# Tianion/topazdb

Hardware: AMD Instinct MI355X
Metric: GiB/s device-resident SSTable block decode+checksum, 4KiB blocks, 1 MI355X (higher is better)
Workload: dtype u8; 1 GPU; 4k: 1048576 blocks/GPU x 4155 B median, 34.0 entries/block, tag 1 (Uncompress); blocks_per_gpu=1048576, input_bytes_per_gpu=4356833280, parallelism=shard1

## Files before the change

### topazdb_amd/csrc/tpz_decode.hip

```cpp

#include <hip/hip_runtime.h>
#include <stdint.h>

#include "tpz_internal.h"
#include "tpz_spill.hip"

namespace tpz {

typedef uint32_t u32;
typedef uint64_t u64;

constexpr int kWave = 64;
#ifdef TPZ_ABL_W20
#ifdef TPZ_ABL_W8
constexpr int kWavesPerWG = 8;
#else
constexpr int kWavesPerWG = 10;
#endif
#else
constexpr int kWavesPerWG = 16;
#endif
constexpr int kWGThreads = kWave * kWavesPerWG;
constexpr u32 kRowShift = 4, kRowBlocks = 1u << kRowShift;
#ifndef TPZ_ROW_AHEAD
// ... 45 lines not shown

__device__ __forceinline__ u32 lane_id() {
  u32 l = __builtin_amdgcn_mbcnt_hi(~0u, __builtin_amdgcn_mbcnt_lo(~0u, 0u));
  asm volatile("" : "+v"(l));
  return l;
}
__device__ __forceinline__ u32 uni(u32 x) { return __builtin_amdgcn_readfirstlane(x); }
__device__ __forceinline__ u64 uni64(u64 x) {
  u32 lo = __builtin_amdgcn_readfirstlane((u32)x), hi = __builtin_amdgcn_readfirstlane((u32)(x >> 32));
  return ((u64)hi << 32) | lo;
}
__device__ __forceinline__ u32 readlane(u32 x, int l) { return __builtin_amdgcn_readlane(x, l); }
template <int CTRL>
__device__ __forceinline__ u32 dpp(u32 x) {
  return (u32)__builtin_amdgcn_update_dpp(0, (int)x, CTRL, 0xF, 0xF, true);
}
constexpr int kRowShr = 0x110;
constexpr int kRowShl = 0x100;

__device__ __forceinline__ u32 lds_u32(const uint8_t* base, u32 a) {
  const u32* p = reinterpret_cast<const u32*>(base + (a & ~3u));
  return __builtin_amdgcn_alignbyte(p[1], p[0], a & 3u);
}
__device__ __forceinline__ u32 lds_be16(const uint8_t* base, u32 a) {
  u32 w = lds_u32(base, a);
  return ((w & 0xFFu) << 8) | ((w >> 8) & 0xFFu);
}
__device__ __forceinline__ u32 bswap32(u32 w) { return __builtin_bswap32(w); }

__device__ __forceinline__ uint4 lds_window16(const uint8_t* base, int x) {
  typedef u32 u32x2 __attribute__((ext_vector_type(2)));
  const u32x2* p = reinterpret_cast<const u32x2*>(base + (x & ~7));
  u32x2 a = p[0], b = p[1], c = p[2];
  asm volatile("" : "+v"(a), "+v"(b), "+v"(c));
  const u32 s = (u32)x & 3u;
  const bool h = ((u32)x & 4u) != 0;
  const u32 s0 = h ? a.y : a.x, s1 = h ? b.x : a.y, s2 = h ? b.y : b.x, s3 = h ? c.x : b.y,
            s4 = h ? c.y : c.x;
  return make_uint4(__builtin_amdgcn_alignbyte(s1, s0, s), __builtin_amdgcn_alignbyte(s2, s1, s),
                    __builtin_amdgcn_alignbyte(s3, s2, s), __builtin_amdgcn_alignbyte(s4, s3, s));
}

#ifdef TPZ_ABL_NOCF
__device__ __forceinline__ u32 tlook(const u32* tab, int id, u32 byte) {
  u32 z = byte;
  asm volatile("" : "+v"(z));
  return tab[id * 256 + (((z & 0x10000u) + __builtin_amdgcn_mbcnt_lo(~0u, 0u)) & 31u)];
}
#elif defined(TPZ_ABL_W20)
__device__ __forceinline__ u32 tlook(const u32* tab, int id, u32 byte) { return tab[(id & 15) * 256 + byte]; }
#else
__device__ __forceinline__ u32 tlook(const u32* tab, int id, u32 byte) { return tab[id * 256 + byte]; }
#endif

__device__ __forceinline__ u32 xor3(u32 a, u32 b, u32 c) { return __builtin_amdgcn_bitop3_b32(a, b, c, 0x96); }

__device__ __forceinline__ u32 slice16(const u32* tab, u32 w0, u32 w1, u32 w2, u32 w3) {
  u32 c = xor3(tlook(tab, 15, w0 & 0xFF), tlook(tab, 14, (w0 >> 8) & 0xFF), tlook(tab, 13, (w0 >> 16) & 0xFF));
  c = xor3(c, tlook(tab, 12, w0 >> 24), tlook(tab, 11, w1 & 0xFF));
  c = xor3(c, tlook(tab, 10, (w1 >> 8) & 0xFF), tlook(tab, 9, (w1 >> 16) & 0xFF));
  c = xor3(c, tlook(tab, 8, w1 >> 24), tlook(tab, 7, w2 & 0xFF));
  c = xor3(c, tlook(tab, 6, (w2 >> 8) & 0xFF), tlook(tab, 5, (w2 >> 16) & 0xFF));
  c = xor3(c, tlook(tab, 4, w2 >> 24), tlook(tab, 3, w3 & 0xFF));
  c = xor3(c, tlook(tab, 2, (w3 >> 8) & 0xFF), tlook(tab, 1, (w3 >> 16) & 0xFF));
  return c ^ tlook(tab, 0, w3 >> 24);
}

__device__ __forceinline__ u32 crc_shift_small(const u32* tab, u32 a, u32 k) {
  u32 r = k >= 4 ? 0u : (a >> (8 * k));
  for (u32 i = 0; i < 4 && i < k; i++) r ^= tlook(tab, (int)(k - 1 - i), (a >> (8 * i)) & 0xFF);
  return r;
}

__device__ __forceinline__ u32 crc_unshift_small(const u32* tab, u32 r, u32 k) {
#ifdef TPZ_ABL_W20
  return r;
#endif
  for (u32 i = 0; i < k; i++) {
    const u32 b = tlook(tab, kCrcInvTable, r >> 24);
    r = ((r ^ tlook(tab, 0, b)) << 8) | b;
  }
  return r;
}

__device__ __forceinline__ u32 gf_mul(u32 a, u32 b) {
  u32 p = 0;
#pragma unroll
  for (int i = 0; i < 32; i++) {
    p ^= (a & (0x80000000u >> i)) ? b : 0u;
    b = (b >> 1) ^ ((b & 1u) ? 0xEDB88320u : 0u);
  }
  return p;
}

__device__ __forceinline__ u32 gf_mul_lane(u32 a, u32 b) {
  u32 p = 0;
#pragma unroll
  for (int i = 0; i < 32; i++) {
    const u32 m = (u32)((int)(a << i) >> 31);
    p ^= b & m;
    b = (b >> 1) ^ (0xEDB88320u & (u32)(-(int)(b & 1u)));
  }
  return p;
}

__device__ __forceinline__ u32 wave_xor(u32 x) {
  x ^= (u32)__builtin_amdgcn_update_dpp(0, (int)x, 0x100 + 1, 0xF, 0xF, true);
  x ^= (u32)__builtin_amdgcn_update_dpp(0, (int)x, 0x100 + 2, 0xF, 0xF, true);
  x ^= (u32)__builtin_amdgcn_update_dpp(0, (int)x, 0x100 + 4, 0xF, 0xF, true);
  x ^= (u32)__builtin_amdgcn_update_dpp(0, (int)x, 0x100 + 8, 0xF, 0xF, true);
  return __builtin_amdgcn_readlane(x, 0) ^ __builtin_amdgcn_readlane(x, 16) ^
         __builtin_amdgcn_readlane(x, 32) ^ __builtin_amdgcn_readlane(x, 48);
}

template <int J>
__device__ __forceinline__ u32 crc_shift(const u32* tab, u32 a) {
  constexpr int b0 = 16 + 4 * J;
  return xor3(tlook(tab, b0, a & 0xFF), tlook(tab, b0 + 1, (a >> 8) & 0xFF),
              tlook(tab, b0 + 2, (a >> 16) & 0xFF)) ^ tlook(tab, b0 + 3, a >> 24);
}

__device__ __forceinline__ uint4 keep_head(uint4 v, u32 k) {
  const u64 lo = (u64)v.y << 32 | v.x, hi = (u64)v.w << 32 | v.z;
  const u64 mlo = k >= 8 ? ~0ull : ((1ull << (8 * k)) - 1);
  const u64 mhi = k >= 16 ? ~0ull : (k <= 8 ? 0ull : ((1ull << (8 * (k - 8))) - 1));
  const u64 a = lo & mlo, b = hi & mhi;
  return make_uint4((u32)a, (u32)(a >> 32), (u32)b, (u32)(b >> 32));
}

__device__ __forceinline__ uint4 zero_head(uint4 v, u32 k) {
  const u64 lo = (u64)v.y << 32 | v.x, hi = (u64)v.w << 32 | v.z;
  const u64 mlo = k >= 8 ? 0ull : (~0ull << (8 * k));
  const u64 mhi = k <= 8 ? ~0ull : (~0ull << (8 * (k - 8)));
  const u64 a = lo & mlo, b = hi & mhi;
  return make_uint4((u32)a, (u32)(a >> 32), (u32)b, (u32)(b >> 32));
}

__device__ __forceinline__ u32 crc_combine(const u32* tab, u32 A) {
  u32 lane = lane_id();
  asm volatile("" : "+v"(lane));
  if ((lane & 1u) == 1u) A = crc_shift<0>(tab, A);
  A ^= dpp<kRowShl + 1>(A);
  if ((lane & 3u) == 2u) A = crc_shift<1>(tab, A);
  A ^= dpp<kRowShl + 2>(A);
  if ((lane & 7u) == 4u) A = crc_shift<2>(tab, A);
  A ^= dpp<kRowShl + 4>(A);
  if ((lane & 15u) == 8u) A = crc_shift<3>(tab, A);
  A ^= dpp<kRowShl + 8>(A);
  if ((lane & 31u) == 16u) A = crc_shift<4>(tab, A);
  if ((lane & 47u) == 32u) A = crc_shift<5>(tab, A);
  return readlane(A, 0) ^ readlane(A, 16) ^ readlane(A, 32) ^ readlane(A, 48);
}

__device__ __forceinline__ u32 wave_crc(const u32* tab, const uint8_t* win, int pb, u32 Pa) {
  typedef u32 u32x4 __attribute__((ext_vector_type(4)));
  const u32 lane = lane_id();
  const u32 S = (Pa + 5119) / 5120;
  u32 A = 0;
  for (u32 r = S; r-- > 0;) {
    const int seg = (int)Pa - 5120 * (int)r - kCrcLaneBytes * (int)(lane + 1);
    u32 c = 0;
    if (seg + kCrcLaneBytes > 0) {
#pragma unroll
      for (int t = 0; t < kCrcLaneBytes / 16; t++) {
        const u32x4 w = *reinterpret_cast<const u32x4*>(win + pb + seg + 16 * t);
        c = slice16(tab, w.x ^ c, w.y, w.z, w.w);
// ... 243 lines not shown
  const u32 vch = V ? (dv + V + 15) >> 4 : 0u;
  D.rk = __builtin_amdgcn_make_buffer_rsrc(o.keys + (kf & ~15ull), (short)0, (int)(16 * kch), 0x00020000);
  D.rv = __builtin_amdgcn_make_buffer_rsrc(o.vals + (vf & ~15ull), (short)0, (int)(16 * vch), 0x00020000);
  const u32 vs = 16 * kch + dv;
  D.rgk = dk | (dk + K) << 16;
  D.rgv = vs | (vs + V) << 16;
  return D;
}
template <bool FLAT>
__device__ __forceinline__ u32 stream_vstart(u32 K, u32 dk, u32 dv) {
  return FLAT ? (K ? (dk + K + 15) & ~15u : 0u) + dv : (K + 15) & ~15u;
}
struct FlatDst {
  static constexpr bool kFlat = true;
  const FlatOut* d;
  __device__ __forceinline__ void put(u32 c, uint4 acc, bool act) const { d->put(c, acc, !act); }
};

template <class Col, class MapT, class S, class D>
__device__ __forceinline__ u32 copy_window(const S& src, const Col& col, const MapT* map, u32 nk,
                                           u32 tot, const D& dst, u32 map_len, u32 w, u32 carry) {
  const u32 nch = (tot + 15) >> 4;
  const u32 lane = lane_id();
  const u32 last = nk ? nk - 1 : 0u;
  const u32 c = 64 * w + lane;
  const u32 x0 = 16 * c;
  const bool act = c < nch;
  u32 j = map[min(c, map_len - 1)];
  j = max(wave_scan_max(act ? j : 0u), carry);
  const u32 carry_out = readlane(j, 63);
  u32 e0, e1;
  int d0, d1;
  col.get2(min(j, last), e0, d0, e1, d1);
  uint4 acc = src(act ? (int)x0 + d0 : 0);
  bool cross = act && j + 1 < nk && e0 < x0 + 16;
  uint4 nx = make_uint4(0, 0, 0, 0);
  if (cross) nx = src((int)x0 + d1);
  if (__ballot(act && e0 <= x0)) {
    while (act && e0 <= x0 && (!D::kFlat || j < last)) {
      j++;
      col.get2(min(j, last), e0, d0, e1, d1);
    }
    acc = src(act ? (int)x0 + d0 : 0);
    cross = act && j + 1 < nk && e0 < x0 + 16;
    if (cross) nx = src((int)x0 + d1);
  }
  if (cross) acc = merge_at(acc, nx, (int)(e0 - x0));
  if (__ballot(cross && e1 < x0 + 16 && j + 2 < nk)) {
    u32 k = j + 1, end = e1;
    while (cross && end < x0 + 16 && k + 1 < nk) {
      const int lo = (int)(end - x0);
      k++;
      int delta;
      col.get(k, end, delta);
      const int hi = min((int)(end - x0), 16);
      const uint4 v = src((int)x0 + delta);
      acc.x = (acc.x & ~byte_mask(lo, hi, 0)) | (v.x & byte_mask(lo, hi, 0));
      acc.y = (acc.y & ~byte_mask(lo, hi, 1)) | (v.y & byte_mask(lo, hi, 1));
      acc.z = (acc.z & ~byte_mask(lo, hi, 2)) | (v.z & byte_mask(lo, hi, 2));
      acc.w = (acc.w & ~byte_mask(lo, hi, 3)) | (v.w & byte_mask(lo, hi, 3));
    }
  }
  dst.put(c, acc, act);
  return carry_out;
}

template <class Col, class MapT, class S, class D>
__device__ __forceinline__ void copy_stream(const S& src, const Col& col, const MapT* map, u32 nk,
                                            u32 tot, const D& dst, u32 map_len) {
  const u32 lane = lane_id();
  const u32 nch = (tot + 15) >> 4;
  const u32 npad = (nch + 7) & ~7u;
  const u32 nw = (npad + 63) >> 6;
#ifdef TPZ_ABL_MEMONLY
  for (u32 c = lane; c < npad; c += 64) dst.put(c, make_uint4(c, 0, 0, 0), c < nch);
  return;
#endif
  u32 carry = 0;
  for (u32 w = 0; w < nw; w++) carry = copy_window(src, col, map, nk, tot, dst, map_len, w, carry);
}

struct PendingCrc {
  u32 live;
  u32 b, st, cnt, stored, k;
  u32 lc;
  u32 early;
};

__device__ __forceinline__ void finish_pending(const u32* tab, const Out& o, PendingCrc& pd) {
  if (!pd.live) return;
  const u32 R = crc_combine(tab, pd.lc);
  const u32 crc = (R == crc_shift_small(tab, ~pd.stored, pd.k)) ? pd.stored
                                                                   : ~crc_unshift_small(tab, R, pd.k);
  const bool ok = crc == pd.stored;
  put_meta(o, pd.b, ok ? pd.st : TPZ_BLOCK_CHECKSUM_MISMATCH, ok ? pd.cnt : 0u, crc);
  pd.live = 0;
}

struct FinishAtExit {
  const u32* tab;
  const Out& o;
  PendingCrc& pd;
  bool on;
  __device__ __forceinline__ ~FinishAtExit() {
    if (on) finish_pending(tab, o, pd);
  }
};

template <int J>
__device__ __forceinline__ bool comb_lane(u32 lane) {
  return J == 0 ? (lane & 1u) == 1u : J == 1 ? (lane & 3u) == 2u : J == 2 ? (lane & 7u) == 4u
       : J == 3 ? (lane & 15u) == 8u : J == 4 ? (lane & 31u) == 16u : (lane & 47u) == 32u;
}
struct CombLv {
  u32 r0, r1, r2, r3;
};
template <int J>
__device__ __forceinline__ CombLv comb_issue(const u32* tab, u32 A) {
  CombLv c;
  if (comb_lane<J>(lane_id())) {
    constexpr int b0 = 16 + 4 * J;
    c.r0 = tlook(tab, b0, A & 0xFF);
    c.r1 = tlook(tab, b0 + 1, (A >> 8) & 0xFF);
    c.r2 = tlook(tab, b0 + 2, (A >> 16) & 0xFF);
    c.r3 = tlook(tab, b0 + 3, A >> 24);
  }
  return c;
}
template <int J>
__device__ __forceinline__ u32 comb_use(u32 A, const CombLv& c) {
  if (comb_lane<J>(lane_id())) A = xor3(c.r0, c.r1, c.r2) ^ c.r3;
  if (J < 4) A ^= dpp<kRowShl + (1 << (J < 4 ? J : 0))>(A);
  return A;
}

__device__ __forceinline__ void comb_finish(const u32* tab, const Out& o, PendingCrc& pd, u32 cA,
                                            u32 want) {
  if (!pd.live) return;
  const u32 R = readlane(cA, 0) ^ readlane(cA, 16) ^ readlane(cA, 32) ^ readlane(cA, 48);
  const u32 crc = R == want ? pd.stored : ~crc_unshift_small(tab, R, pd.k);
  const bool ok = crc == pd.stored;
  put_meta(o, pd.b, ok ? pd.st : TPZ_BLOCK_CHECKSUM_MISMATCH, ok ? pd.cnt : 0u, crc);
  pd.live = 0;
}

struct CrcLane {
  int seg;
  bool act;
  u32 c;
};

__device__ __forceinline__ void crc_step(const u32* tab, const uint8_t* win, int pb, CrcLane& L,
                                         int t) {
  typedef u32 u32x4 __attribute__((ext_vector_type(4)));
  const int a = L.act ? pb + L.seg + 16 * t : -kGuard;
  const u32x4 w = *reinterpret_cast<const u32x4*>(win + a);
  L.c = slice16(tab, w.x ^ L.c, w.y, w.z, w.w);
}
__device__ __forceinline__ u32 crc_lane_value(const u32* tab, const CrcLane& L) { return L.c; }

struct FastWin {
  u32 nk, tot, nch, npad, last;
  __amdgpu_buffer_rsrc_t out;
};

template <bool FLAT, class S>
__device__ __forceinline__ u32 copy_fast(const S& src, const ColSmall& col, const uint16_t* map,
                                         const FastWin& F, const FlatOut& D, u32 w, u32 carry,
                                         u32& rare) {
  const u32 lane = lane_id();
  const u32 c = 64 * w + lane;
  const u32 x0 = 16 * c;
  const bool act = c < F.nch;
  u32 j = map[min(c, (u32)kWaveMapLen - 1)];
  j = max(wave_scan_max(act ? j : 0u), carry);
  const u32 carry_out = readlane(j, 63);
  u32 e0, e1;
  int d0, d1;
  col.get2(min(j, F.last), e0, d0, e1, d1);
  const bool cross = act && j + 1 < F.nk && e0 < x0 + 16;
  uint4 acc = src(act ? (int)x0 + d0 : -kGuard);
  const uint4 nx = src(cross ? (int)x0 + d1 : -kGuard);
  const bool rw = __ballot(act && (e0 <= x0 || (cross && e1 < x0 + 16 && j + 2 < F.nk))) != 0;
  if (rw) rare |= 1u << w;
  if (cross) acc = merge_at(acc, nx, (int)(e0 - x0));
  if (FLAT) {
    D.put(c, acc, rw);
  } else {
    __builtin_amdgcn_raw_buffer_store_b128(__builtin_bit_cast(__attribute__((ext_vector_type(4))) u32, acc),
                                           F.out, rw ? kOob : x0, 0, 0);
  }
  return carry_out;
}

template <bool FLAT, class S>
__device__ __forceinline__ u32 copy_fast3(const S& src, const ColSmall& col, const uint16_t* map,
                                          const FastWin& F, const FlatOut& D, u32 w, u32 carry,
                                          u32& rare) {
  const u32 lane = lane_id();
  const u32 c = 64 * w + lane;
  const u32 x0 = 16 * c;
  const bool act = c < F.nch;
  u32 j = map[min(c, (u32)kWaveMapLen - 1)];
  j = max(wave_scan_max(act ? j : 0u), carry);
  const u32 carry_out = readlane(j, 63);
  u32 e0, e1, e2, e3;
  int d0, d1, d2, d3;
  col.get2(min(j, F.last), e0, d0, e1, d1);
  col.get2(min(j + 2, F.last), e2, d2, e3, d3);
  if (act && e0 <= x0) {
    j++;
    e0 = e1, d0 = d1, e1 = e2, d1 = d2, e2 = e3, d2 = d3;
  }
  const bool b1 = act && j + 1 < F.nk && e0 < x0 + 16;
  const bool b2 = b1 && j + 2 < F.nk && e1 < x0 + 16;
  uint4 acc = src(act ? (int)x0 + d0 : -kGuard);
  const uint4 n1 = src(b1 ? (int)x0 + d1 : -kGuard);
  const uint4 n2 = src(b2 ? (int)x0 + d2 : -kGuard);
  const bool rw = __ballot(act && (e0 <= x0 || (b2 && e2 < x0 + 16 && j + 3 < F.nk))) != 0;
  if (rw) rare |= 1u << w;
  if (b1) acc = merge_at(acc, n1, (int)(e0 - x0));
  if (b2) acc = merge_at(acc, n2, (int)(e1 - x0));
  if (FLAT)
    D.put(c, acc, rw);
  else
    __builtin_amdgcn_raw_buffer_store_b128(__builtin_bit_cast(__attribute__((ext_vector_type(4))) u32, acc),
                                           F.out, rw ? kOob : x0, 0, 0);
  return carry_out;
}

template <bool SHORT, bool FLAT, class S>
__device__ __forceinline__ u32 copy_crc_fused(const u32* tab, const S& src, const ColSmall& col,
                                              const uint16_t* map, u32 nk, u32 tot, uint8_t* dst,
                                              const FlatOut& D, const uint8_t* win, int pb, u32 Pa,
                                              u32 kshift, Stamps& St, u32 w3, const Out& o,
                                              PendingCrc& pd) {
  const u32 lane = lane_id();
  FastWin F;
  F.nk = nk;
  F.tot = tot;
  F.nch = (tot + 15) >> 4;
  F.npad = FLAT ? F.nch : (F.nch + 7) & ~7u;
  F.last = nk ? nk - 1 : 0u;
  F.out = __builtin_amdgcn_make_buffer_rsrc(dst, (short)0, FLAT ? 0 : (int)(F.npad * 16), 0x00020000);
  const u32 nw = (F.npad + 63) >> 6;
  CrcLane L;
  L.seg = (int)Pa - kCrcLaneBytes * (int)(lane + 1);
  L.act = L.seg + kCrcLaneBytes > 0;
  L.c = 0;
  u32 carry = 0, rare = 0, cw[5];
  const bool pl = pd.live != 0;
  u32 cA = pd.lc, want = 0;
  CombLv cl{0u, 0u, 0u, 0u};
  if (pl) {
    cl = comb_issue<0>(tab, cA);
    want = crc_shift_small(tab, ~pd.stored, pd.k);
  }
#pragma unroll
  for (int t = 0; t < 4; t++) {
    cw[t] = carry;
    crc_step(tab, win, pb, L, t);
    carry = (SHORT && (u32)t < w3) ? copy_fast3<FLAT>(src, col, map, F, D, (u32)t, carry, rare)
                                   : copy_fast<FLAT>(src, col, map, F, D, (u32)t, carry, rare);
    if (pl) {
      if (t == 0) { cA = comb_use<0>(cA, cl); cl = comb_issue<1>(tab, cA); }
      if (t == 1) { cA = comb_use<1>(cA, cl); cl = comb_issue<2>(tab, cA); }
      if (t == 2) { cA = comb_use<2>(cA, cl); cl = comb_issue<3>(tab, cA); }
      if (t == 3) { cA = comb_use<3>(cA, cl); cl = comb_issue<4>(tab, cA); }
    }
  }
  cw[4] = carry;
  crc_step(tab, win, pb, L, 4);
  if (pl) {
    cA = comb_use<4>(cA, cl);
    cl = comb_issue<5>(tab, cA);
  }
  if (nw > 4)
    carry = (SHORT && 4u < w3) ? copy_fast3<FLAT>(src, col, map, F, D, 4u, carry, rare)
                               : copy_fast<FLAT>(src, col, map, F, D, 4u, carry, rare);
  if (pl) comb_finish(tab, o, pd, comb_use<5>(cA, cl), want);
  TPZ_STAMP(St, 4);
#ifdef TPZ_ABL_STAMPS
  St.rare += __builtin_popcount(rare);
#endif
  if (rare) {
    for (u32 w = 0; w < nw; w++)
      if (rare & (1u << w)) {
        if (FLAT)
          copy_window(src, col, map, nk, F.tot, FlatDst{&D}, (u32)kWaveMapLen, w, cw[w]);
        else
          copy_window(src, col, map, nk, F.tot, SlotDst{dst, F.npad, F.tot}, (u32)kWaveMapLen, w, cw[w]);
      }
  }
  return crc_lane_value(tab, L);
}

typedef u32 u32x2v __attribute__((ext_vector_type(2)));
typedef u32 u32x4v __attribute__((ext_vector_type(4)));
struct Gath {
  u32 d0, d1, d2, d3, d4;
};
__device__ __forceinline__ Gath gath_issue(const uint8_t* base, int x) {
  const u32* p = reinterpret_cast<const u32*>(base + (x & ~3));
  Gath g;
  g.d0 = p[0];
  g.d1 = p[1];
  g.d2 = p[2];
  g.d3 = p[3];
  g.d4 = p[4];
  return g;
}
__device__ __forceinline__ uint4 gath_finish(Gath g, int x) {
  asm volatile("" : "+v"(g.d0), "+v"(g.d1), "+v"(g.d2), "+v"(g.d3), "+v"(g.d4));
  const u32 s = (u32)x & 3u;
  return make_uint4(__builtin_amdgcn_alignbyte(g.d1, g.d0, s), __builtin_amdgcn_alignbyte(g.d2, g.d1, s),
                    __builtin_amdgcn_alignbyte(g.d3, g.d2, s), __builtin_amdgcn_alignbyte(g.d4, g.d3, s));
}
struct Look16 {
  u32 r[16];
};
__device__ __forceinline__ Look16 look_issue(const u32* tab, u32x4v w, u32 c) {
  Look16 L;
  const u32 w0 = w.x ^ c;
#pragma unroll
  for (int i = 0; i < 4; i++) {
    L.r[i] = tlook(tab, 15 - i, (w0 >> (8 * i)) & 0xFF);
    L.r[4 + i] = tlook(tab, 11 - i, (w.y >> (8 * i)) & 0xFF);
    L.r[8 + i] = tlook(tab, 7 - i, (w.z >> (8 * i)) & 0xFF);
    L.r[12 + i] = tlook(tab, 3 - i, (w.w >> (8 * i)) & 0xFF);
  }
  return L;
}
__device__ __forceinline__ u32 look_xor(const Look16& L) {
  u32 c = xor3(L.r[0], L.r[1], L.r[2]);
  c = xor3(c, L.r[3], L.r[4]);
  c = xor3(c, L.r[5], L.r[6]);
  c = xor3(c, L.r[7], L.r[8]);
  c = xor3(c, L.r[9], L.r[10]);
  c = xor3(c, L.r[11], L.r[12]);
  c = xor3(c, L.r[13], L.r[14]);
  return c ^ L.r[15];
}
#define TPZ_SB() __builtin_amdgcn_sched_barrier(0)

struct PWin {
  u32 m, j;
  u32 e0, e1;
  int d0, d1;
  bool act, cross;
  Gath ga, gn;
};
struct PWin3 {
  u32 e2, e3;
  int d2, d3;
  bool b2;
  Gath g2;
};

struct RegGeom {
  u32 n, KL, VL, db;
};
constexpr u32 kRegShift = 26;
__device__ __forceinline__ u32 reg_recip(u32 d) {
  float f = (float)d;
  asm volatile("" : "+v"(f));
  u32 m = (u32)(__builtin_amdgcn_rcpf(f) * (float)(1u << kRegShift)) + 2u;
  asm volatile("" : "+v"(m));
  return uni(m);
}
__device__ __forceinline__ u32 mul24(u32 a, u32 b) { return (a & 0xFFFFFFu) * (b & 0xFFFFFFu); }
__device__ __forceinline__ u32 reg_div(u32 y, u32 m) {
  const u64 p = (u64)(y & 0x1FFFu) * (u64)(m & 0x7FFFFFu);
  return __builtin_amdgcn_alignbit((u32)(p >> 32), (u32)p, kRegShift) & 0x3FFu;
}

struct RegForm {
  u32 n, KL, VL, kc, vs, S, mk, mv;
  int gap;
  __device__ __forceinline__ RegForm(u32 n_, u32 KL_, u32 VL_) : n(n_), KL(KL_), VL(VL_) {
    kc = n * KL, vs = (kc + 15) & ~15u, S = 4 + KL + VL;
    mk = reg_recip(KL), mv = reg_recip(VL);
    gap = (int)(2 + KL) - (int)vs - (int)((n - 1) * (4 + VL));
  }
  __device__ __forceinline__ void entry(u32 x0, u32 db, bool isk, u32& e0, int& d0, int& d1) const {
    const u32 L = isk ? KL : VL, base = isk ? 0u : vs, T = S - L;
    const u32 j = reg_div(x0 - base, isk ? mk : mv);
    const bool last = j + 1 == n;
    e0 = (!isk && last) ? 0xFFFFu : base + mul24(j + 1, L);
    d0 = (int)((isk ? db + 2 : db + 4 + KL - vs) + mul24(j, T));
    d1 = d0 + ((isk && last) ? gap : (int)T);
  }
  __device__ __forceinline__ void index(u32 w, u32 lane, u32 db, u32& e0, int& d0, int& d1) const {
    const u32 x0 = 16 * (64 * w + lane);
    if (1024 * (w + 1) <= kc) entry(x0, db, true, e0, d0, d1);
    else if (1024 * w >= vs) entry(x0, db, false, e0, d0, d1);
    else entry(x0, db, x0 < kc, e0, d0, d1);
  }
};
constexpr u32 kRegBias = 16, kRegNoChunk = 0x80000000u | (16u << 26);
__device__ __forceinline__ u32 reg_pack(const RegForm& R, u32 w, u32 lane, u32 nch) {
  const u32 c = 64 * w + lane, x0 = 16 * c;
  u32 e0;
  int d0, d1;
  R.entry(x0, 0u, x0 < R.kc, e0, d0, d1);
  const bool cross = e0 < x0 + 16;
  const u32 word = ((x0 + (u32)d0) & 0x1FFFu) |
                   (cross ? (((x0 + (u32)d1 + kRegBias) & 0x1FFFu) << 13) | ((e0 - x0) << 26) : 16u << 26);
  return c < nch ? word : kRegNoChunk;
}
constexpr u32 kRegNone = 0u;
__device__ __forceinline__ u32 reg_key(u32 n, u32 KL, u32 VL) {
  return n == 1 ? 0x80000000u | VL << 13 | KL : n << 24 | VL << 12 | KL;
}
template <bool ON>
struct RegKeyVar {
  u32 key = kRegNone;
  __device__ __forceinline__ u32* ptr() { return &key; }
};
template <>
struct RegKeyVar<false> {
  __device__ __forceinline__ u32* ptr() { return nullptr; }
};
template <bool ON>
struct RegWords {
  u32x4v v;
};
template <>
struct RegWords<false> {};

template <bool FLAT, u32 K3, bool REG = false>
__device__ __forceinline__ u32 copy_crc_piped(const u32* tab, const ColSmall& col,
                                              const uint16_t* map, u32 nk, u32 tot, uint8_t* dst,
                                              const FlatOut& D, const uint8_t* win, int pb, u32 Pa,
                                              const Out& o, PendingCrc& pd, u32 k3n = K3,
                                              const RegGeom G = RegGeom{0u, 0u, 0u, 0u},
                                              const u32x4v rix = u32x4v{0u, 0u, 0u, 0u}) {
  static_assert(!REG || (K3 == 0 && !FLAT), "the regular copy: slotted, no short keys");
  const u32 lane = lane_id();
  FastWin F;
  F.nk = nk;
  F.tot = tot;
  F.nch = (tot + 15) >> 4;
  F.npad = FLAT ? F.nch : (F.nch + 7) & ~7u;
  F.last = nk ? nk - 1 : 0u;
  F.out = __builtin_amdgcn_make_buffer_rsrc(dst, (short)0, FLAT ? 0 : (int)(F.npad * 16), 0x00020000);
  const u32 nw = (F.npad + 63) >> 6;
  const int seg = (int)Pa - kCrcLaneBytes * (int)(lane + 1);
  const bool cact = seg + kCrcLaneBytes > 0;
  const int cbase = cact ? pb + seg : -kGuard;
  auto dread = [&](int t) -> u32x4v {
    return *reinterpret_cast<const u32x4v*>(win + cbase + 16 * t);
  };
  PWin W[4];
  PWin3 W3;
  auto reg_unpack = [&](PWin& P, u32 word) {
    P.e0 = (word >> 26) & 31u;
    P.d0 = (int)word < 0 ? -kGuard : (int)(G.db + (word & 0x1FFFu));
    P.d1 = P.e0 < 16 ? (int)(G.db - kRegBias + ((word >> 13) & 0x1FFFu)) : -kGuard;
    asm volatile("" : "+v"(P.e0), "+v"(P.d0), "+v"(P.d1));
  };
  if constexpr (!REG) {
#pragma unroll
    for (int w = 0; w < 4; w++) {
      const u32 c = 64 * w + lane;
      W[w].act = c < F.nch;
      W[w].m = map[min(c, (u32)kWaveMapLen - 1)];
    }
  }
  u32x4v dA = dread(0);
  u32 cA = pd.lc;
  CombLv cl = comb_issue<0>(tab, cA);
  const u32 want = crc_shift_small(tab, ~pd.stored, pd.k);
  TPZ_SB();
  u32 cw[5];
  cw[0] = 0;
  if (REG) {
    reg_unpack(W[0], rix.x);
    reg_unpack(W[1], rix.y);
    reg_unpack(W[2], rix.z);
    reg_unpack(W[3], rix.w);
  } else {
#pragma unroll
    for (int w = 0; w < 4; w++) W[w].j = wave_scan_max(W[w].act ? W[w].m : 0u);
#pragma unroll
    for (int w = 0; w < 4; w++) {
      W[w].j = max(W[w].j, cw[w]);
      cw[w + 1] = readlane(W[w].j, 63);
    }
#pragma unroll
    for (int w = 0; w < 4; w++) col.get2(min(W[w].j, F.last), W[w].e0, W[w].d0, W[w].e1, W[w].d1);
  }
  if (K3) col.get2(min(W[0].j + 2, F.last), W3.e2, W3.d2, W3.e3, W3.d3);
  cA = comb_use<0>(cA, cl);
  cl = comb_issue<1>(tab, cA);
  TPZ_SB();
  Look16 LK = look_issue(tab, dA, 0u);
  u32x4v dB = dread(1);
  cA = comb_use<1>(cA, cl);
  cl = comb_issue<2>(tab, cA);
  TPZ_SB();
  u32 rare = 0;
  auto gissue = [&](PWin& P, u32 w) {
    if constexpr (REG) {
      P.ga = gath_issue(win, P.d0);
      P.gn = gath_issue(win, P.d1);
      return;
    }
    const u32 x0 = 16 * (64 * w + lane);
    if (w < K3 && w < k3n) {
      if (w > 0) col.get2(min(P.j + 2, F.last), W3.e2, W3.d2, W3.e3, W3.d3);
      if (P.act && P.e0 <= x0) {
        P.j++;
        P.e0 = P.e1, P.d0 = P.d1, P.e1 = W3.e2, P.d1 = W3.d2, W3.e2 = W3.e3, W3.d2 = W3.d3;
      }
      P.cross = P.act && P.j + 1 < F.nk && P.e0 < x0 + 16;
      W3.b2 = P.cross && P.j + 2 < F.nk && P.e1 < x0 + 16;
      if (__ballot(P.act && (P.e0 <= x0 || (W3.b2 && W3.e2 < x0 + 16 && P.j + 3 < F.nk))) != 0)
        rare |= 1u << w;
      W3.g2 = gath_issue(win, W3.b2 ? (int)x0 + W3.d2 : -kGuard);
    } else {
      P.cross = P.act && P.j + 1 < F.nk && P.e0 < x0 + 16;
    }
    P.ga = gath_issue(win, P.act ? (int)x0 + P.d0 : -kGuard);
    P.gn = gath_issue(win, P.cross ? (int)x0 + P.d1 : -kGuard);
  };
  auto finish = [&](PWin& P, u32 w) {
    const u32 c = 64 * w + lane;
    const u32 x0 = 16 * c;
    if constexpr (REG) {
      uint4 acc = gath_finish(P.ga, P.d0);
      const uint4 nx = gath_finish(P.gn, P.d1);
      if (P.e0 < 16) acc = merge_at(acc, nx, (int)P.e0);
      __builtin_amdgcn_raw_buffer_store_b128(__builtin_bit_cast(u32x4v, acc), F.out, x0, 0, 0);
      return;
    }
    const bool rw = w < K3 && w < k3n && (rare & (1u << w));
    uint4 acc = gath_finish(P.ga, P.act ? (int)x0 + P.d0 : -kGuard);
    const uint4 nx = gath_finish(P.gn, P.cross ? (int)x0 + P.d1 : -kGuard);
    if (P.cross) acc = merge_at(acc, nx, (int)(P.e0 - x0));
    if (w < K3 && w < k3n) {
      const uint4 n2 = gath_finish(W3.g2, W3.b2 ? (int)x0 + W3.d2 : -kGuard);
      if (W3.b2) acc = merge_at(acc, n2, (int)(P.e1 - x0));
    }
    if (FLAT)
      D.put(c, acc, rw);
    else
      __builtin_amdgcn_raw_buffer_store_b128(__builtin_bit_cast(u32x4v, acc), F.out, rw ? kOob : x0, 0, 0);
  };
  gissue(W[0], 0);
  cA = comb_use<2>(cA, cl);
  cl = comb_issue<3>(tab, cA);
  TPZ_SB();
  u32 crc = 0;
  crc = look_xor(LK);
  LK = look_issue(tab, dB, crc);
  dA = dread(2);
  cA = comb_use<3>(cA, cl);
  cl = comb_issue<4>(tab, cA);
  TPZ_SB();
  finish(W[0], 0);
  gissue(W[1], 1);
  cA = comb_use<4>(cA, cl);
  cl = comb_issue<5>(tab, cA);
  TPZ_SB();
  crc = look_xor(LK);
  LK = look_issue(tab, dA, crc);
  dB = dread(3);
  cA = comb_use<5>(cA, cl);
  comb_finish(tab, o, pd, cA, want);
  TPZ_SB();
  finish(W[1], 1);
  gissue(W[2], 2);
  TPZ_SB();
  crc = look_xor(LK);
  LK = look_issue(tab, dB, crc);
  dA = dread(4);
  TPZ_SB();
  finish(W[2], 2);
  gissue(W[3], 3);
  TPZ_SB();
  crc = look_xor(LK);
  LK = look_issue(tab, dA, crc);
  TPZ_SB();
  finish(W[3], 3);
  TPZ_SB();
  crc = look_xor(LK);
  if (nw > 4) {
    if (REG) {
      const RegForm R(G.n, G.KL, G.VL);
      const u32 x0 = 16 * (256 + lane);
      u32 e0;
      int d0, d1;
      R.index(4u, lane, G.db, e0, d0, d1);
      const bool act = 256 + lane < F.nch, cross = act && e0 < x0 + 16;
      W[0].e0 = cross ? e0 - x0 : 16u;
      W[0].d0 = act ? (int)x0 + d0 : -kGuard;
      W[0].d1 = cross ? (int)x0 + d1 : -kGuard;
      gissue(W[0], 4u);
      finish(W[0], 4u);
    } else {
      (void)copy_fast<FLAT>(Src16{win}, col, map, F, D, 4u, cw[4], rare);
    }
  }
  if (!REG && rare) {
    for (u32 w = 0; w < nw; w++)
      if (rare & (1u << w)) {
        if (FLAT)
          copy_window(Src16{win}, col, map, nk, F.tot, FlatDst{&D}, (u32)kWaveMapLen, w, cw[w]);
        else
          copy_window(Src16{win}, col, map, nk, F.tot, SlotDst{dst, F.npad, F.tot}, (u32)kWaveMapLen, w, cw[w]);
      }
  }
  return crc;
}


__device__ __forceinline__ u32 crc_prepare(uint8_t* win, u32 a0, u32 P) {
  const u32 lane = lane_id();
  const u32 k = ((a0 + P + 15) & ~15u) - (a0 + P);
  if (lane < 4) win[a0 + lane] ^= 0xFFu;
  if (lane < 16) win[a0 + P + lane] = 0;
  __builtin_amdgcn_wave_barrier();
  return k;
}

template <class Col, class MapT, int kMapLen, bool BIG, bool FLAT = false>
__device__ __forceinline__ void decode_block(const u32* tab, uint8_t* win, const Col& col,
                                             MapT* map, u32 a0, u32 len, u32 b, u64 ext_b,
                                             const Out& o, u32 kshift, Stamps& S, PendingCrc& pd,
                                             u64 kf = 0, u64 vf = 0, u64 ef = 0,
                                             const Out* o_lds = nullptr, u32* rk = nullptr) {
  const u32 lane = lane_id();
  const u32 tag = win[(int)(a0 + len) - 1];
  const u32 stored = bswap32(lds_u32(win, len >= 5 ? a0 + len - 5 : a0));
  const u32 n = lds_be16(win, a0);
  const u32 dk = (u32)kf & 15u, dv = (u32)vf & 15u;
  u32 e_off = 0, e_kl = 0;
  bool e_ok = false;
  if (!BIG) {
    e_off = lds_be16(win, a0 + 2 + 2 * lane);
    const u32 Pn = len - 5, db0 = a0 + 2 + 2 * n;
    e_ok = len >= 7 && lane < n && Pn >= 2 + 2 * n && e_off + 2 <= Pn - 2 - 2 * n;
    e_kl = lds_be16(win, e_ok ? db0 + e_off : a0);
  }
  RegWords<!BIG && !FLAT> rix;
  if (pd.early) finish_pending(tab, o, pd);
  FinishAtExit fin{tab, o, pd, true};
  if (len == 0) { put_meta(o, b, TPZ_BLOCK_EMPTY, 0, 0); return; }
  if (tag == 0 || tag > 3) { put_meta(o, b, TPZ_BLOCK_BAD_TAG, 0, 0); return; }
  if (tag != 1) { put_meta(o, b, TPZ_BLOCK_UNSUPPORTED_CODEC, 0, 0); return; }
  if (len - 1 < 4) { put_meta(o, b, TPZ_BLOCK_MALFORMED, 0, 0); return; }
  const u32 P = len - 5;
  const int pb = (int)a0;
  u32 st = TPZ_BLOCK_OK, cnt = n;
  bool fuse = false;
  bool f_short = false;
  u32 f_w3 = 0;
  u32 f_nk = 0, f_tot = 0;
  uint8_t* f_dst = nullptr;
  FlatOut fo;
  if (P < 2 || P < 2 + 2 * n) {
    st = TPZ_BLOCK_MALFORMED;
    cnt = 0;
  } else if (!BIG && n > kWaveMaxN) {
    const Out& oc = o_lds ? *o_lds : o;
    if (FLAT) defer_to(oc.spill_list, oc.spill_count, b);
    else defer_to(oc.defer_list, oc.defer_count, b);
    return;
  } else {
    const u32 db = a0 + 2 + 2 * n;
    const u32 dl = P - 2 - 2 * n;
    const bool slots_fit = FLAT || 6u * n <= len;
    uint2* ends_g = reinterpret_cast<uint2*>(o.ends) + uni64((FLAT || o.efirst) ? ef : entry_base(ext_b, b));
    const u32 n_pad = o.efirst ? n : (n + 15) & ~15u;
    u32 r_vl = 0;
    bool r_ok = false;
    if constexpr (!BIG && !FLAT) {
      r_ok = e_ok && e_off + 4 + e_kl <= dl;
      if (r_ok) { r_vl = lds_be16(win, db + e_off + 2 + e_kl); r_ok = e_off + 4 + e_kl + r_vl <= dl; }
      const u32 KL = readlane(e_kl, 0), VL = readlane(r_vl, 0), es = 4 + KL + VL;
      bool reg = n != 0 && KL >= 16 && VL >= 16 && P >= 4 && slots_fit &&
                 !__ballot(lane < n && !(r_ok && e_off == mul24(lane, es) && e_kl == KL && r_vl == VL));
      for (u32 g0 = 64; reg && g0 < n; g0 += 64) {
        const u32 i = g0 + lane;
        bool same = true;
        if (i < n) {
          const u32 off = lds_be16(win, a0 + 2 + 2 * i);
          same = off == mul24(i, es) && off + 4 + KL + VL <= dl;
          if (same) same = lds_be16(win, db + off) == KL && lds_be16(win, db + off + 2 + KL) == VL;
        }
        reg = !__ballot(!same);
      }
      const u32 kc = n * KL, vc = n * VL, vs = stream_vstart<false>(kc, 0u, 0u);
      if (reg && vs + vc <= len + 2u) {
        for (u32 g0 = 0; g0 < n; g0 += 64) {
          const u32 i = g0 + lane;
          __builtin_amdgcn_raw_buffer_store_b64(
              __builtin_bit_cast(__attribute__((ext_vector_type(2))) u32,
                                 i < n ? make_uint2(mul24(i + 1, KL), mul24(i + 1, VL)) : make_uint2(0, 0)),
              whole_rsrc(ends_g), i < n_pad ? 8 * i : kOob, 0, 0);
        }
        TPZ_STAMP(S, 2);
        TPZ_STAMP(S, 3);
        const u32 key = reg_key(n, KL, VL);
        rix.v = *reinterpret_cast<const u32x4v*>(reinterpret_cast<const uint8_t*>(col.t) + 16 * lane);
        if (*rk != key) {
          const RegForm R(n, KL, VL);
          const u32 nch = (vs + vc + 15) >> 4;
#pragma nounroll
          for (u32 w = 0; w < 4; w++) col.t[4 * lane + w] = reg_pack(R, w, lane, nch);
          rix.v = *reinterpret_cast<const u32x4v*>(reinterpret_cast<const uint8_t*>(col.t) + 16 * lane);
          *rk = key;
        }
        __builtin_amdgcn_wave_barrier();
        const u32 k = crc_prepare(win, a0, P);
        fin.on = false;
        const u32 lc = copy_crc_piped<false, 0u, true>(
            tab, *reinterpret_cast<const ColSmall*>(&col), reinterpret_cast<const uint16_t*>(map),
            2 * n, vs + vc, o.data + slot_base(ext_b, b), fo, win, pb, P + k, o, pd, 0u,
            RegGeom{n, KL, VL, db}, rix.v);
        pd = PendingCrc{1u, b, st, cnt, stored, k, lc, 0u};
        return;
      }
      *rk = kRegNone;
    }
    {
      constexpr u32 per = 16 / sizeof(MapT);
      const u32 nz = min((u32)kMapLen, ((len >> 4) + 3 + per - 1) / per * per);
      for (u32 i = lane; i < nz / per; i += 64)
        reinterpret_cast<uint4*>(map)[i] = make_uint4(0, 0, 0, 0);
    }
    u32 ktot = 0, knz_all = 0;
    if (n > 64) {
      for (u32 g0 = 0; g0 < n; g0 += 64) {
        const u32 i = g0 + lane;
        u32 kl = 0;
        if (i < n) {
          const u32 off = lds_be16(win, a0 + 2 + 2 * i);
          if (off + 2 <= dl) {
            kl = lds_be16(win, db + off);
            if (off + 4 + kl > dl) kl = 0;
          }
        }
        knz_all += __builtin_popcountll(__ballot(kl != 0));
        ktot += readlane(wave_scan_incl(kl), 63);
      }
    }
    u32 kc = 0, vc = 0, knz = 0, vnz = 0;
    bool bad = false, short_k = false, short_v = false;
    for (u32 g0 = 0; g0 < n; g0 += 64) {
      const u32 i = g0 + lane;
      const bool act = i < n;
      u32 off = 0, kl = 0, vl = 0;
      bool ok = true;
      if (act) {
        if (!BIG && !FLAT && g0 == 0) {
          off = e_off;
          kl = e_kl;
          vl = r_vl;
          ok = r_ok;
        } else {
          if (!BIG && g0 == 0) {
            off = e_off;
            ok = e_ok;
            if (ok) { kl = e_kl; ok = off + 4 + kl <= dl; }
          } else {
            off = lds_be16(win, a0 + 2 + 2 * i);
            ok = off + 2 <= dl;
            if (ok) { kl = lds_be16(win, db + off); ok = off + 4 + kl <= dl; }
          }
          if (ok) { vl = lds_be16(win, db + off + 2 + kl); ok = off + 4 + kl + vl <= dl; }
        }
        if (!ok) kl = vl = 0;
      }
      bad |= __ballot(act && !ok) != 0;
      short_k |= __ballot(kl != 0 && kl < 16) != 0;
      short_v |= __ballot(vl != 0 && vl < 16) != 0;
      const u32 ki = wave_scan_incl(kl) + kc;
      const u32 vi = wave_scan_incl(vl) + vc;
      const u64 kmask = __ballot(kl != 0), vmask = __ballot(vl != 0);
      if (n <= 64) {
        ktot = readlane(ki, 63);
        knz_all = __builtin_popcountll(kmask);
      }
      const u32 vs = stream_vstart<FLAT>(ktot, dk, dv);
      __builtin_amdgcn_raw_buffer_store_b64(
          __builtin_bit_cast(__attribute__((ext_vector_type(2))) u32,
                             act ? make_uint2(ki, vi) : make_uint2(0, 0)),
          whole_rsrc(ends_g), (slots_fit && i < n_pad) ? 8 * i : kOob, 0, 0);
      if (act && slots_fit) {
        if (kl) {
          const u32 m = knz + lanes_below(kmask);
          const u32 ke = ki + dk;
          col.put(m, ke, (int)(db + off + 2) - (int)(ke - kl));
          if (((ke + 15) >> 4) < (u32)kMapLen) map[(ke + 15) >> 4] = (MapT)(m + 1);
        }
        if (vl) {
          const u32 m = knz_all + vnz + lanes_below(vmask);
          const u32 ve = vs + vi;
          col.put(m, ve, (int)(db + off + 4 + kl) - (int)(ve - vl));
          if (((ve + 15) >> 4) < (u32)kMapLen) map[(ve + 15) >> 4] = (MapT)(m + 1);
        }
      }
      knz += __builtin_popcountll(kmask);
      vnz += __builtin_popcountll(vmask);
      kc = readlane(ki, 63);
      vc = readlane(vi, 63);
    }

    const u32 vs = stream_vstart<FLAT>(kc, dk, dv);
    TPZ_STAMP(S, 2);
    if (bad || !slots_fit || vs + vc > len + (FLAT ? 47u : 2u)) {
      const Out& oc = o_lds ? *o_lds : o;
      defer_to(oc.spill_list, oc.spill_count, b);
      return;
    } else {
      if (BIG) {
        asm volatile("s_waitcnt vmcnt(0)" ::: "memory");
        __builtin_amdgcn_fence(__ATOMIC_RELEASE, "workgroup");
      }
      __builtin_amdgcn_wave_barrier();
      const u32 tot = FLAT ? (vc ? vs + vc : (kc ? dk + kc : 0u)) : vs + vc;
#ifndef TPZ_ABL_NOCOPY
#if !defined(TPZ_ABL_NOCRC) && !defined(TPZ_ABL_MEMONLY)
#ifdef TPZ_ABL_UNFUSED
      if (false) {
#else
      if (!BIG && P >= 4) {
#endif
        fuse = true;
        f_w3 = short_v ? 5u : (short_k ? (((FLAT ? dk : 0u) + kc + 15) / 16 + 63) / 64 : 0u);
        f_short = f_w3 != 0;
        f_nk = knz + vnz;
        f_tot = tot;
        f_dst = FLAT ? nullptr : o.data + slot_base(ext_b, b);
        if (FLAT) fo = flat_out(o, kf, vf, kc, vc);
      } else
#endif
      if (FLAT) {
        fo = flat_out(o, kf, vf, kc, vc);
        copy_stream(Src16{win}, col, map, knz + vnz, tot, FlatDst{&fo}, (u32)kMapLen);
      } else {
        const u32 nch = (tot + 15) >> 4;
        copy_stream(Src16{win}, col, map, knz + vnz, tot,
                    SlotDst{o.data + slot_base(ext_b, b), (nch + 7) & ~7u, tot}, (u32)kMapLen);
      }
#endif
    }
    TPZ_STAMP(S, 3);
  }
  __builtin_amdgcn_wave_barrier();
  u32 crc;
  if (P >= 4) {
    const u32 k = crc_prepare(win, a0, P);
#if defined(TPZ_ABL_NOCRC) || defined(TPZ_ABL_MEMONLY)
    crc = stored;
#else
    u32 R;
    if (!BIG && fuse) {
      u32 lc;
      fin.on = false;
      if (!f_short) {
        lc = copy_crc_piped<FLAT, 0u>(tab, *reinterpret_cast<const ColSmall*>(&col),
                                         reinterpret_cast<const uint16_t*>(map), f_nk, f_tot, f_dst,
                                         fo, win, pb, P + k, o, pd);
      } else if (f_w3 <= 2u) {
        lc = copy_crc_piped<FLAT, 2u>(tab, *reinterpret_cast<const ColSmall*>(&col),
                                      reinterpret_cast<const uint16_t*>(map), f_nk, f_tot, f_dst,
                                      fo, win, pb, P + k, o, pd, FLAT ? 2u : f_w3);
        f_short = false;
      } else
      {
        lc = f_short
          ? copy_crc_fused<true, FLAT>(tab, Src16{win}, *reinterpret_cast<const ColSmall*>(&col),
                                       reinterpret_cast<const uint16_t*>(map), f_nk, f_tot, f_dst,
                                       fo, win, pb, P + k, kshift, S, f_w3, o, pd)
          : copy_crc_fused<false, FLAT>(tab, Src16{win}, *reinterpret_cast<const ColSmall*>(&col),
                                        reinterpret_cast<const uint16_t*>(map), f_nk, f_tot, f_dst,
                                        fo, win, pb, P + k, kshift, S, 5u, o, pd);
      }
      pd = PendingCrc{1u, b, st, cnt, stored, k, lc, f_short ? 1u : 0u};
      return;
    } else {
        R = wave_crc(tab, win, pb, P + k);
    }
    if constexpr (BIG)
      crc = (R == crc_shift_small(tab, ~stored, k)) ? stored : ~crc_unshift_small(tab, R, k);
    else
      crc = (R == crc_shift_small(tab, ~stored, k)) ? stored : ~crc_unshift_small(tab, R, k);
#endif
  } else {
    u32 c = 0xFFFFFFFFu;
    for (u32 i = 0; i < P; i++) {
      c ^= win[a0 + i];
      for (int k = 0; k < 8; k++) c = (c >> 1) ^ (0xEDB88320u & (0u - (c & 1u)));
    }
    crc = ~c;
  }
  if (crc != stored) {
    st = TPZ_BLOCK_CHECKSUM_MISMATCH;
    cnt = 0;
  }
  TPZ_STAMP(S, 6);
  put_meta(o, b, st, cnt, crc);
}

__device__ __forceinline__ void load_tables(u32* tab, const u32* gtab, int bytes = kTableBytes) {
  const uint4* s = reinterpret_cast<const uint4*>(gtab);
  uint4* d = reinterpret_cast<uint4*>(tab);
  for (int i = threadIdx.x; i < bytes / 16; i += blockDim.x) d[i] = s[i];
  __syncthreads();
}

__device__ __forceinline__ __amdgpu_buffer_rsrc_t window_rsrc(const uint8_t* src, u64 src_bytes,
                                                               u64 wstart) {
  u64 rem = src_bytes > wstart ? src_bytes - wstart : 0;
  if (rem > 0x7FFFFFF0ull) rem = 0x7FFFFFF0ull;
  return __builtin_amdgcn_make_buffer_rsrc((void*)(src + wstart), (short)0, (int)rem, 0x00020000);
}

__device__ __forceinline__ void fix_tail(uint4& v, const uint8_t* src, u64 piece, u64 src_bytes) {
  const bool straddle = piece + 16 > src_bytes && piece < src_bytes;
  if (__ballot(straddle)) {
    u32 w[4] = {0, 0, 0, 0};
#pragma unroll
    for (u32 k = 0; k < 16; k++) {
      const u64 a = piece + k;
      const u32 byte = src[a < src_bytes ? a : src_bytes - 1];
      w[k >> 2] |= (a < src_bytes ? byte : 0u) << (8 * (k & 3));
    }
    v.x = straddle ? w[0] : v.x;
    v.y = straddle ? w[1] : v.y;
    v.z = straddle ? w[2] : v.z;
    v.w = straddle ? w[3] : v.w;
  }
}

struct Params {
  u64* big_scratch;
  u64* spill_used;
  const uint8_t* src;
  const u64* ext;
  u64 src_bytes;
  u32 n_blocks;
  const u32* crc_tables;
  Out out;
  u32 xp[kBigSuper];
  u32 lane_shift[64];
  u32 chunk_shift;
  u32* row_ctr;
  u32* err;
};


template <class T>
__device__ __forceinline__ T const_load(const T* base, u64 i) {
  return reinterpret_cast<const __attribute__((address_space(4))) T*>(reinterpret_cast<uintptr_t>(base))[i];
}

#ifdef TPZ_ABL_ROWLATE
__device__ __noinline__ void rowlate_delay(const Params& p, u32 wid, u32 point) {
  const u32 rows = (p.n_blocks + kRowBlocks - 1) / kRowBlocks;
  const u32 ctr = __hip_atomic_load(p.row_ctr, __ATOMIC_RELAXED, __HIP_MEMORY_SCOPE_AGENT);
  const bool late = point == 0 ? (wid & 1u) != 0 : (wid & 3u) == 2;
  if (late && ctr + 2 * gridDim.x >= rows)
    for (int i = 0; i < 30; i++) __builtin_amdgcn_s_sleep(127);
}
#endif
#ifdef TPZ_ABL_ONCHIP
constexpr u32 kOnchipMask = 4095;
#endif
template <bool FLAT, u32 CS>
// ... 700 lines not shown
```

Baseline: 2486 GiB/s.

## Fold stored checksum into CRC stream so verification compares residue to zero

Appends the inverted stored CRC (plus zero padding) to the CRC input, either written into the LDS window or injected via DPP and bitop3 into the last two slice-by-16 steps. A matching block then yields residue zero, so the per-block crc_shift_small expected-value computation disappears from the hot path. The actual CRC is recovered by an unshift only on mismatch. The pending record is packed tighter (cnt and k share one field), and the header word is loaded once to rebuild the leading complemented bytes. This adds lane-shuffle and bit-manipulation work in the tail steps, and every padding, shift and lane-mask choice has to be exactly right for correctness.

```diff
diff --git a/topazdb_amd/csrc/tpz_decode.hip b/topazdb_amd/csrc/tpz_decode.hip
--- a/topazdb_amd/csrc/tpz_decode.hip
+++ b/topazdb_amd/csrc/tpz_decode.hip
@@ -151,6 +151,29 @@
   }
   return r;
 }
+
+__device__ __forceinline__ u32 crc_actual(const u32* tab, u32 R, u32 stored, u32 k) {
+  return stored ^ crc_unshift_small(tab, R, 4u + k);
+}
+struct CrcResidue {
+  u32 stored, k;
+  __device__ __forceinline__ CrcResidue(u32 stored_, u32 k_) : stored(stored_), k(k_) {}
+  __device__ __forceinline__ u32 into3(u32 w) const {
+    const u32 d = k >= 13u ? ~stored << (8u * (16u - k)) : 0u;
+    return __builtin_amdgcn_bitop3_b32(w, lane_id() == 0 ? ~0u : 0u, d, 0x78);
+  }
+  __device__ __forceinline__ u32 lanes4() const {
+    const u32 lane = lane_id();
+    const int t = min(max((int)(12u - k) - (int)lane, -4), 4);
+    const u64 x = ((u64)(~stored) << 32) >> ((8u * (u32)(4 - t)) & 63u);
+    return (lane & ~12u) == 0 ? (u32)x : 0u;
+  }
+  template <int J>
+  __device__ __forceinline__ static u32 into4(u32 w, u32 r) {
+    constexpr int ctrl = J == 0 ? 0xE4 : kRowShl + 4 * J;
+    return w ^ (u32)__builtin_amdgcn_update_dpp(0, (int)r, ctrl, 0x1, 0x1, true);
+  }
+};
 
 __device__ __forceinline__ u32 gf_mul(u32 a, u32 b) {
   u32 p = 0;
@@ -560,7 +583,7 @@
 
 struct PendingCrc {
   u32 live;
-  u32 b, st, cnt, stored, k;
+  u32 b, st, ck, stored;
   u32 lc;
   u32 early;
 };
@@ -568,10 +591,9 @@
 __device__ __forceinline__ void finish_pending(const u32* tab, const Out& o, PendingCrc& pd) {
   if (!pd.live) return;
   const u32 R = crc_combine(tab, pd.lc);
-  const u32 crc = (R == crc_shift_small(tab, ~pd.stored, pd.k)) ? pd.stored
-                                                                   : ~crc_unshift_small(tab, R, pd.k);
-  const bool ok = crc == pd.stored;
-  put_meta(o, pd.b, ok ? pd.st : TPZ_BLOCK_CHECKSUM_MISMATCH, ok ? pd.cnt : 0u, crc);
+  const bool ok = R == 0;
+  const u32 crc = ok ? pd.stored : crc_actual(tab, R, pd.stored, pd.ck >> 16);
+  put_meta(o, pd.b, ok ? pd.st : TPZ_BLOCK_CHECKSUM_MISMATCH, ok ? pd.ck & 0xFFFFu : 0u, crc);
   pd.live = 0;
 }
 
@@ -612,13 +634,12 @@
   return A;
 }
 
-__device__ __forceinline__ void comb_finish(const u32* tab, const Out& o, PendingCrc& pd, u32 cA,
-                                            u32 want) {
+__device__ __forceinline__ void comb_finish(const u32* tab, const Out& o, PendingCrc& pd, u32 cA) {
   if (!pd.live) return;
   const u32 R = readlane(cA, 0) ^ readlane(cA, 16) ^ readlane(cA, 32) ^ readlane(cA, 48);
-  const u32 crc = R == want ? pd.stored : ~crc_unshift_small(tab, R, pd.k);
-  const bool ok = crc == pd.stored;
-  put_meta(o, pd.b, ok ? pd.st : TPZ_BLOCK_CHECKSUM_MISMATCH, ok ? pd.cnt : 0u, crc);
+  const bool ok = R == 0;
+  const u32 crc = ok ? pd.stored : crc_actual(tab, R, pd.stored, pd.ck >> 16);
+  put_meta(o, pd.b, ok ? pd.st : TPZ_BLOCK_CHECKSUM_MISMATCH, ok ? pd.ck & 0xFFFFu : 0u, crc);
   pd.live = 0;
 }
 
@@ -633,6 +654,24 @@
   typedef u32 u32x4 __attribute__((ext_vector_type(4)));
   const int a = L.act ? pb + L.seg + 16 * t : -kGuard;
   const u32x4 w = *reinterpret_cast<const u32x4*>(win + a);
+  L.c = slice16(tab, w.x ^ L.c, w.y, w.z, w.w);
+}
+template <int T>
+__device__ __forceinline__ void crc_step_tail(const u32* tab, const uint8_t* win, int pb, CrcLane& L,
+                                              const CrcResidue& Z) {
+  static_assert(T == 3 || T == 4, "the range's last two pieces");
+  typedef u32 u32x4 __attribute__((ext_vector_type(4)));
+  const int a = L.act ? pb + L.seg + 16 * T : -kGuard;
+  u32x4 w = *reinterpret_cast<const u32x4*>(win + a);
+  if (T == 3) {
+    w.w = Z.into3(w.w);
+  } else {
+    const u32 zr = Z.lanes4();
+    w.x = CrcResidue::into4<0>(w.x, zr);
+    w.y = CrcResidue::into4<1>(w.y, zr);
+    w.z = CrcResidue::into4<2>(w.z, zr);
+    w.w = CrcResidue::into4<3>(w.w, zr);
+  }
   L.c = slice16(tab, w.x ^ L.c, w.y, w.z, w.w);
 }
 __device__ __forceinline__ u32 crc_lane_value(const u32* tab, const CrcLane& L) { return L.c; }
@@ -712,7 +751,7 @@
                                               const uint16_t* map, u32 nk, u32 tot, uint8_t* dst,
                                               const FlatOut& D, const uint8_t* win, int pb, u32 Pa,
                                               u32 kshift, Stamps& St, u32 w3, const Out& o,
-                                              PendingCrc& pd) {
+                                              PendingCrc& pd, const CrcResidue& Z) {
   const u32 lane = lane_id();
   FastWin F;
   F.nk = nk;
@@ -728,16 +767,14 @@
   L.c = 0;
   u32 carry = 0, rare = 0, cw[5];
   const bool pl = pd.live != 0;
-  u32 cA = pd.lc, want = 0;
+  u32 cA = pd.lc;
   CombLv cl{0u, 0u, 0u, 0u};
-  if (pl) {
-    cl = comb_issue<0>(tab, cA);
-    want = crc_shift_small(tab, ~pd.stored, pd.k);
-  }
+  if (pl) cl = comb_issue<0>(tab, cA);
 #pragma unroll
   for (int t = 0; t < 4; t++) {
     cw[t] = carry;
-    crc_step(tab, win, pb, L, t);
+    if (t < 3) crc_step(tab, win, pb, L, t);
+    else crc_step_tail<3>(tab, win, pb, L, Z);
     carry = (SHORT && (u32)t < w3) ? copy_fast3<FLAT>(src, col, map, F, D, (u32)t, carry, rare)
                                    : copy_fast<FLAT>(src, col, map, F, D, (u32)t, carry, rare);
     if (pl) {
@@ -748,7 +785,7 @@
     }
   }
   cw[4] = carry;
-  crc_step(tab, win, pb, L, 4);
+  crc_step_tail<4>(tab, win, pb, L, Z);
   if (pl) {
     cA = comb_use<4>(cA, cl);
     cl = comb_issue<5>(tab, cA);
@@ -756,7 +793,7 @@
   if (nw > 4)
     carry = (SHORT && 4u < w3) ? copy_fast3<FLAT>(src, col, map, F, D, 4u, carry, rare)
                                : copy_fast<FLAT>(src, col, map, F, D, 4u, carry, rare);
-  if (pl) comb_finish(tab, o, pd, comb_use<5>(cA, cl), want);
+  if (pl) comb_finish(tab, o, pd, comb_use<5>(cA, cl));
   TPZ_STAMP(St, 4);
 #ifdef TPZ_ABL_STAMPS
   St.rare += __builtin_popcount(rare);
@@ -910,8 +947,8 @@
 __device__ __forceinline__ u32 copy_crc_piped(const u32* tab, const ColSmall& col,
                                               const uint16_t* map, u32 nk, u32 tot, uint8_t* dst,
                                               const FlatOut& D, const uint8_t* win, int pb, u32 Pa,
-                                              const Out& o, PendingCrc& pd, u32 k3n = K3,
-                                              const RegGeom G = RegGeom{0u, 0u, 0u, 0u},
+                                              const Out& o, PendingCrc& pd, const CrcResidue& Z,
+                                              u32 k3n = K3, const RegGeom G = RegGeom{0u, 0u, 0u, 0u},
                                               const u32x4v rix = u32x4v{0u, 0u, 0u, 0u}) {
   static_assert(!REG || (K3 == 0 && !FLAT), "the regular copy: slotted, no short keys");
   const u32 lane = lane_id();
@@ -948,7 +985,6 @@
   u32x4v dA = dread(0);
   u32 cA = pd.lc;
   CombLv cl = comb_issue<0>(tab, cA);
-  const u32 want = crc_shift_small(tab, ~pd.stored, pd.k);
   TPZ_SB();
   u32 cw[5];
   cw[0] = 0;
@@ -1045,12 +1081,13 @@
   LK = look_issue(tab, dA, crc);
   dB = dread(3);
   cA = comb_use<5>(cA, cl);
-  comb_finish(tab, o, pd, cA, want);
+  comb_finish(tab, o, pd, cA);
   TPZ_SB();
   finish(W[1], 1);
   gissue(W[2], 2);
   TPZ_SB();
   crc = look_xor(LK);
+  dB.w = Z.into3(dB.w);
   LK = look_issue(tab, dB, crc);
   dA = dread(4);
   TPZ_SB();
@@ -1058,6 +1095,11 @@
   gissue(W[3], 3);
   TPZ_SB();
   crc = look_xor(LK);
+  const u32 zr = Z.lanes4();
+  dA.x = CrcResidue::into4<0>(dA.x, zr);
+  dA.y = CrcResidue::into4<1>(dA.y, zr);
+  dA.z = CrcResidue::into4<2>(dA.z, zr);
+  dA.w = CrcResidue::into4<3>(dA.w, zr);
   LK = look_issue(tab, dA, crc);
   TPZ_SB();
   finish(W[3], 3);
@@ -1093,11 +1135,14 @@
 }
 
 
-__device__ __forceinline__ u32 crc_prepare(uint8_t* win, u32 a0, u32 P) {
+constexpr u32 kCrcMaxRange = (15u + (kWaveMaxLen - 5u) + 4u + 15u) & ~15u;
+static_assert(kCrcMaxRange <= (u32)kWinBytes, "the CRC's range ends inside the window");
+static_assert(kCrcMaxRange <= 64u * kCrcLaneBytes && kCrcLaneBytes == 5 * 16, "one run of five steps per lane");
+__device__ __forceinline__ u32 crc_prepare(uint8_t* win, u32 a0, u32 P, u32 hw) {
   const u32 lane = lane_id();
-  const u32 k = ((a0 + P + 15) & ~15u) - (a0 + P);
-  if (lane < 4) win[a0 + lane] ^= 0xFFu;
-  if (lane < 16) win[a0 + P + lane] = 0;
+  const u32 k = (0u - (a0 + P + 4u)) & 15u;
+  if (lane < 4) win[a0 + lane] = (uint8_t)(~hw >> (8u * lane));
+  if (lane < max(16u, 4u + k)) win[a0 + P + lane] = 0;
   __builtin_amdgcn_wave_barrier();
   return k;
 }
@@ -1111,7 +1156,8 @@
   const u32 lane = lane_id();
   const u32 tag = win[(int)(a0 + len) - 1];
   const u32 stored = bswap32(lds_u32(win, len >= 5 ? a0 + len - 5 : a0));
-  const u32 n = lds_be16(win, a0);
+  const u32 hw = lds_u32(win, a0);
+  const u32 n = ((hw & 0xFFu) << 8) | ((hw >> 8) & 0xFFu);
   const u32 dk = (u32)kf & 15u, dv = (u32)vf & 15u;
   u32 e_off = 0, e_kl = 0;
   bool e_ok = false;
@@ -1191,13 +1237,13 @@
           *rk = key;
         }
         __builtin_amdgcn_wave_barrier();
-        const u32 k = crc_prepare(win, a0, P);
+        const u32 k = crc_prepare(win, a0, P, hw);
         fin.on = false;
         const u32 lc = copy_crc_piped<false, 0u, true>(
             tab, *reinterpret_cast<const ColSmall*>(&col), reinterpret_cast<const uint16_t*>(map),
-            2 * n, vs + vc, o.data + slot_base(ext_b, b), fo, win, pb, P + k, o, pd, 0u,
-            RegGeom{n, KL, VL, db}, rix.v);
-        pd = PendingCrc{1u, b, st, cnt, stored, k, lc, 0u};
+            2 * n, vs + vc, o.data + slot_base(ext_b, b), fo, win, pb, P + 4 + k, o, pd,
+            CrcResidue(stored, k), 0u, RegGeom{n, KL, VL, db}, rix.v);
+        pd = PendingCrc{1u, b, st, cnt | k << 16, stored, lc, 0u};
         return;
       }
       *rk = kRegNone;
@@ -1205,8 +1251,10 @@
     {
       constexpr u32 per = 16 / sizeof(MapT);
       const u32 nz = min((u32)kMapLen, ((len >> 4) + 3 + per - 1) / per * per);
+      u32 z = 0;
+      asm volatile("" : "+v"(z));
       for (u32 i = lane; i < nz / per; i += 64)
-        reinterpret_cast<uint4*>(map)[i] = make_uint4(0, 0, 0, 0);
+        reinterpret_cast<uint4*>(map)[i] = make_uint4(z, z, z, z);
     }
     u32 ktot = 0, knz_all = 0;
     if (n > 64) {
@@ -1330,7 +1378,8 @@
   __builtin_amdgcn_wave_barrier();
   u32 crc;
   if (P >= 4) {
-    const u32 k = crc_prepare(win, a0, P);
+    const u32 k = crc_prepare(win, a0, P, hw);
+    const CrcResidue Z(stored, k);
 #if defined(TPZ_ABL_NOCRC) || defined(TPZ_ABL_MEMONLY)
     crc = stored;
 #else
@@ -1341,31 +1390,30 @@
       if (!f_short) {
         lc = copy_crc_piped<FLAT, 0u>(tab, *reinterpret_cast<const ColSmall*>(&col),
                                          reinterpret_cast<const uint16_t*>(map), f_nk, f_tot, f_dst,
-                                         fo, win, pb, P + k, o, pd);
+                                         fo, win, pb, P + 4 + k, o, pd, Z);
       } else if (f_w3 <= 2u) {
         lc = copy_crc_piped<FLAT, 2u>(tab, *reinterpret_cast<const ColSmall*>(&col),
                                       reinterpret_cast<const uint16_t*>(map), f_nk, f_tot, f_dst,
-                                      fo, win, pb, P + k, o, pd, FLAT ? 2u : f_w3);
+                                      fo, win, pb, P + 4 + k, o, pd, Z, FLAT ? 2u : f_w3);
         f_short = false;
       } else
       {
         lc = f_short
           ? copy_crc_fused<true, FLAT>(tab, Src16{win}, *reinterpret_cast<const ColSmall*>(&col),
                                        reinterpret_cast<const uint16_t*>(map), f_nk, f_tot, f_dst,
-                                       fo, win, pb, P + k, kshift, S, f_w3, o, pd)
+                                       fo, win, pb, P + 4 + k, kshift, S, f_w3, o, pd, Z)
           : copy_crc_fused<false, FLAT>(tab, Src16{win}, *reinterpret_cast<const ColSmall*>(&col),
                                         reinterpret_cast<const uint16_t*>(map), f_nk, f_tot, f_dst,
-                                        fo, win, pb, P + k, kshift, S, 5u, o, pd);
-      }
-      pd = PendingCrc{1u, b, st, cnt, stored, k, lc, f_short ? 1u : 0u};
+                                        fo, win, pb, P + 4 + k, kshift, S, 5u, o, pd, Z);
+      }
+      pd = PendingCrc{1u, b, st, cnt | k << 16, stored, lc, f_short ? 1u : 0u};
       return;
     } else {
-        R = wave_crc(tab, win, pb, P + k);
-    }
-    if constexpr (BIG)
-      crc = (R == crc_shift_small(tab, ~stored, k)) ? stored : ~crc_unshift_small(tab, R, k);
-    else
-      crc = (R == crc_shift_small(tab, ~stored, k)) ? stored : ~crc_unshift_small(tab, R, k);
+      if (lane < 4) win[a0 + P + lane] = (uint8_t)(~stored >> (8u * lane));
+      __builtin_amdgcn_wave_barrier();
+      R = wave_crc(tab, win, pb, P + 4 + k);
+    }
+    crc = R == 0 ? stored : crc_actual(tab, R, stored, k);
 #endif
   } else {
     u32 c = 0xFFFFFFFFu;
```

Result: no change. 2482 GiB/s (-0.2%).
